# lukefleed/two-pass-lanczos

Measured on AMD Instinct MI355X. Metric: Lanczos iterations/sec + SpMV GB/s (vs HBM roofline), 500k-arc KKT k=500, higher is better.
Workload: dtype f64

## Files before the change

two-pass-lanczos_amd/csrc/tpl_k_p2_fused.hip:

```cpp
#include "tpl_klaunch.h"

namespace tpl {

constexpr int kHubAhead = 8;

struct FusedP2Args {
  const int32_t* h_row;
  const int32_t* h_ent;
  const double* h_val;
  int32_t n_open, n_hub;
  double* ycache;
  const double* rec;
  const int32_t* flags;
  const double* v1;
  double* x;
  int64_t n;
  int32_t n_long;
  int32_t steps;
  const void* s_col;
  const void* s_val;
  const int32_t* s_cbase;
  const int32_t* c_base;
  const int32_t* c_width;
  int32_t n_short, n_chunks, s_width, val_i8, s_col16;
};

__device__ __forceinline__ int fused_steps(const FusedP2Args& a) {
  if (a.steps > 0) return a.steps;
  return a.flags[1] || a.flags[4] ? 0 : a.flags[2];
}

struct StepRec {
  double beta_sub, alpha, invb, ycoef;
};
__device__ __forceinline__ StepRec rec_fields(double cv) {
  return {readlane_f64(cv, 0), readlane_f64(cv, 1), readlane_f64(cv, 2), readlane_f64(cv, 3)};
}
__device__ __forceinline__ void fused_step_r(double s, const StepRec& r, double& vc, double& vp,
                                             double& xv) {
  double w = s - r.beta_sub * vp;
  w = w - r.alpha * vc;
  const double vn = w * r.invb;
  xv = xv + r.ycoef * vn;
  vp = vc;
  vc = vn;
}
__device__ __forceinline__ void fused_step(double s, double cv, double& vc, double& vp, double& xv) {
  fused_step_r(s, rec_fields(cv), vc, vp, xv);
}

constexpr uint32_t kLaneOff = 0x80000000u;
__device__ __forceinline__ void st_cache_row(double* row, int nl, uint32_t off, double v) {
  typedef uint32_t u32x2 __attribute__((ext_vector_type(2)));
  const __amdgpu_buffer_rsrc_t r = __builtin_amdgcn_make_buffer_rsrc(row, 0, nl * 8, 0x00020000);
  u32x2 d;
  d.x = (uint32_t)__double2loint(v);
  d.y = (uint32_t)__double2hiint(v);
  __builtin_amdgcn_raw_buffer_store_b64(d, r, off, 0, 0);
}

enum HubMode { kHubLong, kHubLds, kHubWave };
constexpr int kWave = 64;
template <HubMode MODE>
__device__ __forceinline__ void hub_chain(const FusedP2Args& a, double (*vh)[kTPB], int last,
                                          int lc, bool writes, bool open,
                                          const int (&ent)[kFusedWidth],
                                          const double (&av)[kFusedWidth], double& vc, double& vp,
                                          double& xv) {
  const int t = threadIdx.x;
  const int nl = a.n_long;
  double yb[kHubAhead], cb[kHubAhead];
#pragma unroll
  for (int u = 0; u < kHubAhead; ++u) {
    const int jj = clampi(1 + u, last);
    yb[u] = a.ycache[(size_t)(jj - 1) * nl + lc];
    cb[u] = a.rec[8 * (size_t)jj + (t & 7)];
  }
  const uint32_t soff = writes ? (uint32_t)lc * 8u : kLaneOff;
  auto step = [&](int j, double s, double cv) {
    st_cache_row(a.ycache + (size_t)(j - 1) * nl, nl, soff, vc);
    if (MODE == kHubLds) {
      double* vb = vh[j & 1];
      vb[t] = vc;
      __syncthreads();
      if (open) {
        s = 0.0;
#pragma unroll
        for (int k = 0; k < kFusedWidth; ++k) {
          const double prod = av[k] * vb[ent[k] < 0 ? 0 : ent[k]];
          s = s + (ent[k] >= 0 ? prod : -0.0);
        }
      }
    }
    if (MODE == kHubWave) {
      double so = 0.0;
#pragma unroll
      for (int k = 0; k < kFusedWidth; ++k) {
        const double prod = av[k] * __shfl(vc, ent[k] < 0 ? 0 : ent[k], kWave);
        so = so + (ent[k] >= 0 ? prod : -0.0);
      }
      s = open ? so : s;
    }
    fused_step(s, cv, vc, vp, xv);
  };
  const int nblk = last / kHubAhead;
  int j0 = 1;
  if (nblk > 0) __builtin_amdgcn_s_waitcnt(0x0F70);
  for (int b = 0; b < nblk; ++b, j0 += kHubAhead) {
#pragma unroll
    for (int u = 0; u < kHubAhead; ++u) {
      const int j = j0 + u;
      step(j, yb[u], cb[u]);
      __builtin_amdgcn_sched_barrier(0);
      const int jn = clampi(j + kHubAhead, last);
      yb[u] = a.ycache[(size_t)(jn - 1) * nl + lc];
      cb[u] = a.rec[8 * (size_t)jn + (t & 7)];
    }
  }
  const int rem = last - nblk * kHubAhead;
#pragma unroll
  for (int u = 0; u < kHubAhead - 1; ++u) {
    if (u >= rem) break;
    step(j0 + u, yb[u], cb[u]);
  }
}

__global__ __launch_bounds__(kTPB) void k_p2_hub(FusedP2Args a) {
  __shared__ double vh[2][kTPB];
  const int steps = fused_steps(a);
  if (steps < 2) return;
  const int last = steps - 1;
  const int t = threadIdx.x;
  const int nl = a.n_long;
  const int64_t first_long = a.n - nl;
  const int n_lb = (nl + kTPB - 1) / kTPB;
  const bool hub = (int)blockIdx.x >= n_lb;
  bool live, open = false;
  int lc;
  int64_t row;
  int ent[kFusedWidth];
  double av[kFusedWidth];
#pragma unroll
  for (int k = 0; k < kFusedWidth; ++k) {
    ent[k] = -1;
    av[k] = 0.0;
  }
  if (hub) {
    live = t < a.n_hub;
    open = t < a.n_open;
    row = a.h_row[clampi(t, a.n_hub - 1)];
    lc = open ? 0 : clampi((int)(row - first_long), nl - 1);
    if (open) {
#pragma unroll
      for (int k = 0; k < kFusedWidth; ++k) {
        ent[k] = a.h_ent[t * kFusedWidth + k];
        av[k] = a.h_val[t * kFusedWidth + k];
      }
    }
  } else {
    const int l = blockIdx.x * kTPB + t;
    lc = clampi(l, nl - 1);
    row = first_long + lc;
    live = l < nl;
    for (int h = a.n_open; h < a.n_hub; ++h) live = live && a.h_row[h] != (int32_t)row;
  }
  double vc = a.v1[row], vp = 0.0, xv = a.x[row];
  if (hub && a.n_hub <= kWave) {
    if (t >= kWave) return;
    hub_chain<kHubWave>(a, vh, last, lc, live && !open, open, ent, av, vc, vp, xv);
  } else if (hub) {
    hub_chain<kHubLds>(a, vh, last, lc, live && !open, open, ent, av, vc, vp, xv);
  } else {
    hub_chain<kHubLong>(a, vh, last, lc, live, false, ent, av, vc, vp, xv);
  }
  if (live) st_out(a.x + row, xv);
}

__device__ __forceinline__ int fused_col(const FusedP2Args& a, int e, int cbase) {
  if (a.s_col16) {
    const int off = reinterpret_cast<const uint16_t*>(a.s_col)[e];
    return off == 0xFFFF ? -1 : cbase + off;
  }
  return reinterpret_cast<const int32_t*>(a.s_col)[e];
}
__device__ __forceinline__ double fused_val(const FusedP2Args& a, int e) {
  if (a.val_i8) return (double)reinterpret_cast<const int8_t*>(a.s_val)[e];
  return reinterpret_cast<const double*>(a.s_val)[e];
}

constexpr int kRowsGroup = 4;
constexpr int kRowsThreads = kTPB * kRowsGroup;
constexpr int kRowsDepth = 2;

template <int W, int NL>
__global__ __launch_bounds__(kRowsThreads) void k_p2_rows(FusedP2Args a) {
  extern __shared__ double lds[];
  constexpr int NLC = (NL + kRowsGroup - 1) / kRowsGroup;
  constexpr int D = kRowsDepth;
  const int steps = fused_steps(a);
  if (steps < 2) return;
  const int last = steps - 1;
  const int tw = threadIdx.x;
  const int t = tw % kTPB;
  const int chunk_w = blockIdx.x * kRowsGroup + tw / kTPB;
  const bool have = chunk_w < a.n_chunks;
  const int chunk = have ? chunk_w : a.n_chunks - 1;
  const int nl = a.n_long;
  const int first_long = (int)(a.n - nl);
  const int wc = a.s_width > 0 ? a.s_width : a.c_width[chunk];
  const int base = a.s_width > 0 ? chunk * kChunkRows * a.s_width : a.c_base[chunk];
  const bool packed = a.s_width > 0 && packed_chunk_width(a.s_width);
  const int cbase = a.s_col16 ? a.s_cbase[chunk] : 0;
  int row[kRowsPerThread];
  bool live[kRowsPerThread];
  int li[kRowsPerThread][W];
  double av[kRowsPerThread][W];
  double vc[kRowsPerThread], vp[kRowsPerThread], xv[kRowsPerThread];
#pragma unroll
  for (int q = 0; q < kRowsPerThread; ++q) {
    const int p = chunk * kChunkRows + q * kTPB + t;
    live[q] = have && p < a.n_short;
    row[q] = clampi(p, a.n_short - 1);
#pragma unroll
    for (int k = 0; k < W; ++k) {
      const int kc = clampi(k, wc - 1);
      const int e = wc <= 0 ? 0
                    : packed ? base + t * (kRowsPerThread * wc) + q * wc + kc
                             : base + kc * kChunkRows + q * kTPB + t;
      const int c = fused_col(a, e, cbase);
      av[q][k] = fused_val(a, e);
      int idx = -1;
      if (k < wc && c >= 0) {
        if (c >= first_long) idx = c - first_long;
        else if (c == row[q]) idx = -2;
        else live[q] = false;
      }
      li[q][k] = idx;
    }
    vc[q] = a.v1[row[q]];
    vp[q] = 0.0;
    xv[q] = a.x[row[q]];
  }
  double st[D][NLC], cvr[D];
#pragma unroll
  for (int d = 0; d < D; ++d) {
    const int jj = clampi(1 + d, last);
#pragma unroll
    for (int u = 0; u < NLC; ++u)
      st[d][u] = a.ycache[(size_t)(jj - 1) * nl + clampi(tw + u * kRowsThreads, nl - 1)];
    cvr[d] = a.rec[8 * (size_t)jj + (tw & 7)];
  }
  auto step = [&](int j, int d, auto refill) {
    double* vb = lds + (j & 1) * nl;
#pragma unroll
    for (int u = 0; u < NLC; ++u)
      if (u < NLC - 1 || tw + u * kRowsThreads < nl) vb[tw + u * kRowsThreads] = st[d][u];
    const StepRec r = rec_fields(cvr[d]);
    if (decltype(refill)::value) {
      __builtin_amdgcn_sched_barrier(0);
      const int jn = clampi(j + D, last);
#pragma unroll
      for (int u = 0; u < NLC; ++u)
        st[d][u] = a.ycache[(size_t)(jn - 1) * nl + clampi(tw + u * kRowsThreads, nl - 1)];
      cvr[d] = a.rec[8 * (size_t)jn + (tw & 7)];
    }
    __syncthreads();
#pragma unroll
    for (int q = 0; q < kRowsPerThread; ++q) {
      double s = 0.0;
#pragma unroll
      for (int k = 0; k < W; ++k) {
        const double g = vb[li[q][k] < 0 ? 0 : li[q][k]];
        const double prod = av[q][k] * (li[q][k] == -2 ? vc[q] : g);
        s = s + (li[q][k] != -1 ? prod : -0.0);
      }
      fused_step_r(s, r, vc[q], vp[q], xv[q]);
    }
  };
  const int nblk = last / D;
  int j0 = 1;
  if (nblk > 0) __builtin_amdgcn_s_waitcnt(0x0F70);
  for (int b = 0; b < nblk; ++b, j0 += D) {
#pragma unroll
    for (int d = 0; d < D; ++d) step(j0 + d, d, std::true_type{});
  }
  const int rem = last - nblk * D;
#pragma unroll
  for (int d = 0; d < D - 1; ++d) {
    if (d >= rem) break;
    step(j0 + d, d, std::false_type{});
  }
#pragma unroll
  for (int q = 0; q < kRowsPerThread; ++q)
    if (live[q]) st_out(a.x + row[q], xv[q]);
}

namespace launch {

static FusedP2Args fused_args(const CsrDev& A, const DevState& S, const double* ycache,
                              const double* v1, double* x, int steps) {
  FusedP2Args a{};
  a.ycache = const_cast<double*>(ycache);
  a.rec = S.p2c;
  a.flags = S.flags;
  a.v1 = v1;
  a.x = x;
  a.n = A.n;
  a.n_long = A.n_long;
  a.steps = steps;
  a.s_col = A.s_col;
  a.s_val = A.s_val;
  a.s_cbase = A.s_cbase;
  a.c_base = A.c_base;
  a.c_width = A.c_width;
  a.n_short = A.n_short;
  a.n_chunks = A.n_chunks;
  a.s_width = A.s_width;
  a.val_i8 = A.val_i8;
  a.s_col16 = A.s_col16;
  return a;
}

hipError_t p2_fused_hub(const CsrDev& A, const DevState& S, const FusedP2Dev& H, double* ycache,
                        const double* v1, double* x, int steps, hipStream_t s) {
  if (A.n_long <= 0 || !A.s_identity || H.n_hub > kFusedHubMax || H.n_open > H.n_hub)
    return hipErrorInvalidConfiguration;
  FusedP2Args a = fused_args(A, S, ycache, v1, x, steps);
  a.h_row = H.h_row;
  a.h_ent = H.h_ent;
  a.h_val = H.h_val;
  a.n_open = H.n_open;
  a.n_hub = H.n_hub;
  const int grid = (A.n_long + kTPB - 1) / kTPB + (H.n_hub > 0 ? 1 : 0);
  hipLaunchKernelGGL(k_p2_hub, dim3(grid), dim3(kTPB), 0, s, a);
  return hipGetLastError();
}

template <int W, int... NLs>
static bool rows_nl(int nloads, const FusedP2Args& a, int grid, size_t lds, hipStream_t s,
                    std::integer_sequence<int, NLs...>) {
  auto one = [&](auto NL) {
    if (nloads != decltype(NL)::value + 1) return false;
    hipLaunchKernelGGL((k_p2_rows<W, decltype(NL)::value + 1>), dim3(grid), dim3(kRowsThreads),
                       lds, s, a);
    return true;
  };
  return (one(std::integral_constant<int, NLs>{}) || ...);
}

hipError_t p2_fused_rows(const CsrDev& A, const DevState& S, const double* ycache,
                         const double* v1, double* x, int steps, hipStream_t s) {
  if (A.n_long <= 0 || A.n_long > kFusedLongMax || !A.s_identity)
    return hipErrorInvalidConfiguration;
  if (A.n_chunks <= 0) return hipSuccess;
  const FusedP2Args a = fused_args(A, S, ycache, v1, x, steps);
  const size_t lds = 2 * (size_t)A.n_long * sizeof(double);
  const int nloads = (A.n_long + kTPB - 1) / kTPB;
  constexpr auto nls = std::make_integer_sequence<int, kFusedLongMax / kTPB>{};
  const int w = A.s_width > 0 ? A.s_width : kFusedWidth;
  const int grid = (A.n_chunks + kRowsGroup - 1) / kRowsGroup;
  bool ok = false;
  switch (w) {
    case 1: ok = rows_nl<1>(nloads, a, grid, lds, s, nls); break;
    case 2: ok = rows_nl<2>(nloads, a, grid, lds, s, nls); break;
    case 3: ok = rows_nl<3>(nloads, a, grid, lds, s, nls); break;
    case 4: ok = rows_nl<4>(nloads, a, grid, lds, s, nls); break;
    default: break;
  }
  return ok ? hipGetLastError() : hipErrorInvalidConfiguration;
}

}
}
```

Before: 92400.

## Batch several Lanczos steps per LDS sync and specialize hub gather by width

```diff
diff --git a/two-pass-lanczos_amd/csrc/tpl_k_p2_fused.hip b/two-pass-lanczos_amd/csrc/tpl_k_p2_fused.hip
--- a/two-pass-lanczos_amd/csrc/tpl_k_p2_fused.hip
+++ b/two-pass-lanczos_amd/csrc/tpl_k_p2_fused.hip
@@ -33,8 +33,10 @@
 struct StepRec {
   double beta_sub, alpha, invb, ycoef;
 };
-__device__ __forceinline__ StepRec rec_fields(double cv) {
-  return {readlane_f64(cv, 0), readlane_f64(cv, 1), readlane_f64(cv, 2), readlane_f64(cv, 3)};
+__device__ __forceinline__ StepRec rec_scalar(const double* rec, int j) {
+  typedef const double __attribute__((address_space(4))) cdouble;
+  cdouble* p = (cdouble*)(uintptr_t)(rec + 8 * (size_t)j);
+  return {p[0], p[1], p[2], p[3]};
 }
 __device__ __forceinline__ void fused_step_r(double s, const StepRec& r, double& vc, double& vp,
                                              double& xv) {
@@ -45,9 +47,6 @@
   vp = vc;
   vc = vn;
 }
-__device__ __forceinline__ void fused_step(double s, double cv, double& vc, double& vp, double& xv) {
-  fused_step_r(s, rec_fields(cv), vc, vp, xv);
-}
 
 constexpr uint32_t kLaneOff = 0x80000000u;
 __device__ __forceinline__ void st_cache_row(double* row, int nl, uint32_t off, double v) {
@@ -59,9 +58,10 @@
   __builtin_amdgcn_raw_buffer_store_b64(d, r, off, 0, 0);
 }
 
-enum HubMode { kHubLong, kHubLds, kHubWave };
+enum HubMode { kHubLong, kHubLds, kHubWave, kHubLanes };
 constexpr int kWave = 64;
-template <HubMode MODE>
+constexpr int kHubLanesMax = 3;
+template <HubMode MODE, int WM = kFusedWidth, int NH = 0>
 __device__ __forceinline__ void hub_chain(const FusedP2Args& a, double (*vh)[kTPB], int last,
                                           int lc, bool writes, bool open,
                                           const int (&ent)[kFusedWidth],
@@ -69,15 +69,21 @@
                                           double& xv) {
   const int t = threadIdx.x;
   const int nl = a.n_long;
-  double yb[kHubAhead], cb[kHubAhead];
+  double yb[kHubAhead];
+  double2 ra[kHubAhead], rb[kHubAhead];
+  auto load_rec = [&](int u, int jj) {
+    const double2* p = reinterpret_cast<const double2*>(a.rec + 8 * (size_t)jj);
+    ra[u] = p[0];
+    rb[u] = p[1];
+  };
 #pragma unroll
   for (int u = 0; u < kHubAhead; ++u) {
     const int jj = clampi(1 + u, last);
     yb[u] = a.ycache[(size_t)(jj - 1) * nl + lc];
-    cb[u] = a.rec[8 * (size_t)jj + (t & 7)];
+    load_rec(u, jj);
   }
   const uint32_t soff = writes ? (uint32_t)lc * 8u : kLaneOff;
-  auto step = [&](int j, double s, double cv) {
+  auto step = [&](int j, double s, const StepRec& r) {
     st_cache_row(a.ycache + (size_t)(j - 1) * nl, nl, soff, vc);
     if (MODE == kHubLds) {
       double* vb = vh[j & 1];
@@ -86,7 +92,7 @@
       if (open) {
         s = 0.0;
 #pragma unroll
-        for (int k = 0; k < kFusedWidth; ++k) {
+        for (int k = 0; k < WM; ++k) {
           const double prod = av[k] * vb[ent[k] < 0 ? 0 : ent[k]];
           s = s + (ent[k] >= 0 ? prod : -0.0);
         }
@@ -95,14 +101,30 @@
     if (MODE == kHubWave) {
       double so = 0.0;
 #pragma unroll
-      for (int k = 0; k < kFusedWidth; ++k) {
+      for (int k = 0; k < WM; ++k) {
         const double prod = av[k] * __shfl(vc, ent[k] < 0 ? 0 : ent[k], kWave);
         so = so + (ent[k] >= 0 ? prod : -0.0);
       }
       s = open ? so : s;
     }
-    fused_step(s, cv, vc, vp, xv);
-  };
+    if (MODE == kHubLanes) {
+      double bm[NH > 0 ? NH : 1];
+#pragma unroll
+      for (int m = 0; m < NH; ++m) bm[m] = readlane_f64(vc, m);
+      double so = 0.0;
+#pragma unroll
+      for (int k = 0; k < WM; ++k) {
+        double g = bm[0];
+#pragma unroll
+        for (int m = 1; m < NH; ++m) g = ent[k] == m ? bm[m] : g;
+        const double prod = av[k] * g;
+        so = so + (ent[k] >= 0 ? prod : -0.0);
+      }
+      s = open ? so : s;
+    }
+    fused_step_r(s, r, vc, vp, xv);
+  };
+  auto rec_of = [&](int u) { return StepRec{ra[u].x, ra[u].y, rb[u].x, rb[u].y}; };
   const int nblk = last / kHubAhead;
   int j0 = 1;
   if (nblk > 0) __builtin_amdgcn_s_waitcnt(0x0F70);
@@ -110,18 +132,29 @@
 #pragma unroll
     for (int u = 0; u < kHubAhead; ++u) {
       const int j = j0 + u;
-      step(j, yb[u], cb[u]);
+      step(j, yb[u], rec_of(u));
       __builtin_amdgcn_sched_barrier(0);
       const int jn = clampi(j + kHubAhead, last);
       yb[u] = a.ycache[(size_t)(jn - 1) * nl + lc];
-      cb[u] = a.rec[8 * (size_t)jn + (t & 7)];
+      load_rec(u, jn);
     }
   }
   const int rem = last - nblk * kHubAhead;
 #pragma unroll
   for (int u = 0; u < kHubAhead - 1; ++u) {
     if (u >= rem) break;
-    step(j0 + u, yb[u], cb[u]);
+    step(j0 + u, yb[u], rec_of(u));
+  }
+}
+
+template <int NH, typename... Args>
+__device__ __forceinline__ void hub_wave(int wm, Args&&... args) {
+  constexpr HubMode M = NH > 0 ? kHubLanes : kHubWave;
+  switch (wm) {
+    case 1: return hub_chain<M, 1, NH>(args...);
+    case 2: return hub_chain<M, 2, NH>(args...);
+    case 3: return hub_chain<M, 3, NH>(args...);
+    default: return hub_chain<M, kFusedWidth, NH>(args...);
   }
 }
 
@@ -167,7 +200,17 @@
   double vc = a.v1[row], vp = 0.0, xv = a.x[row];
   if (hub && a.n_hub <= kWave) {
     if (t >= kWave) return;
-    hub_chain<kHubWave>(a, vh, last, lc, live && !open, open, ent, av, vc, vp, xv);
+    int wm = 1;
+#pragma unroll
+    for (int k = 1; k < kFusedWidth; ++k)
+      if (__builtin_amdgcn_ballot_w64(ent[k] >= 0) != 0) wm = k + 1;
+    const bool wr = live && !open;
+    static_assert(kHubLanesMax == 3, "the cases below");
+    switch (a.n_hub <= kHubLanesMax ? a.n_hub : 0) {
+      case 2: hub_wave<2>(wm, a, vh, last, lc, wr, open, ent, av, vc, vp, xv); break;
+      case 3: hub_wave<3>(wm, a, vh, last, lc, wr, open, ent, av, vc, vp, xv); break;
+      default: hub_wave<0>(wm, a, vh, last, lc, wr, open, ent, av, vc, vp, xv); break;
+    }
   } else if (hub) {
     hub_chain<kHubLds>(a, vh, last, lc, live && !open, open, ent, av, vc, vp, xv);
   } else {
@@ -191,12 +234,22 @@
 constexpr int kRowsGroup = 4;
 constexpr int kRowsThreads = kTPB * kRowsGroup;
 constexpr int kRowsDepth = 2;
+constexpr int kRowsStepsMax = 3;
+constexpr int kRowsGatherMax = 12;
+
+constexpr int rows_block_steps(int NL) {
+  const int fit = (64 * 1024) / (2 * kTPB * NL * (int)sizeof(double));
+  return fit < kRowsStepsMax ? fit : kRowsStepsMax;
+}
 
 template <int W, int NL>
 __global__ __launch_bounds__(kRowsThreads) void k_p2_rows(FusedP2Args a) {
   extern __shared__ double lds[];
-  constexpr int NLC = (NL + kRowsGroup - 1) / kRowsGroup;
+  constexpr int S = rows_block_steps(NL);
+  constexpr int NLB = (S * NL + kRowsGroup - 1) / kRowsGroup;
   constexpr int D = kRowsDepth;
+  constexpr int kBuf = S * kTPB * NL;
+  static_assert(S >= 1 && 2 * kBuf * sizeof(double) <= 64 * 1024, "two buffers in one workgroup's LDS");
   const int steps = fused_steps(a);
   if (steps < 2) return;
   const int last = steps - 1;
@@ -241,54 +294,126 @@
     vp[q] = 0.0;
     xv[q] = a.x[row[q]];
   }
-  double st[D][NLC], cvr[D];
-#pragma unroll
-  for (int d = 0; d < D; ++d) {
-    const int jj = clampi(1 + d, last);
-#pragma unroll
-    for (int u = 0; u < NLC; ++u)
-      st[d][u] = a.ycache[(size_t)(jj - 1) * nl + clampi(tw + u * kRowsThreads, nl - 1)];
-    cvr[d] = a.rec[8 * (size_t)jj + (tw & 7)];
-  }
-  auto step = [&](int j, int d, auto refill) {
-    double* vb = lds + (j & 1) * nl;
-#pragma unroll
-    for (int u = 0; u < NLC; ++u)
-      if (u < NLC - 1 || tw + u * kRowsThreads < nl) vb[tw + u * kRowsThreads] = st[d][u];
-    const StepRec r = rec_fields(cvr[d]);
+  const int bw = S * nl;
+  bool any_live = false, lane_clean = true;
+#pragma unroll
+  for (int q = 0; q < kRowsPerThread; ++q) {
+    any_live = any_live || live[q];
+#pragma unroll
+    for (int k = 0; k < W; ++k) lane_clean = lane_clean && (!live[q] || k >= wc || li[q][k] >= 0);
+  }
+  const int wcu = __builtin_amdgcn_readfirstlane(wc);
+  const bool idle = __builtin_amdgcn_ballot_w64(any_live) == 0;
+  const bool clean = __builtin_amdgcn_ballot_w64(!lane_clean) == 0;
+  int lx[kRowsPerThread][W];
+#pragma unroll
+  for (int q = 0; q < kRowsPerThread; ++q)
+#pragma unroll
+    for (int k = 0; k < W; ++k) lx[q][k] = (li[q][k] < 0 ? 0 : li[q][k]) * S;
+  double st[D][NLB];
+  int wofs[NLB];
+#pragma unroll
+  for (int u = 0; u < NLB; ++u) {
+    const int i = tw + u * kRowsThreads;
+    int sb = 0;
+#pragma unroll
+    for (int s = 1; s < S; ++s) sb += i >= s * nl ? 1 : 0;
+    wofs[u] = (i - sb * nl) * S + sb;
+  }
+  uint32_t cb[NLB];
+#pragma unroll
+  for (int u = 0; u < NLB; ++u) cb[u] = 8u * (uint32_t)clampi(tw + u * kRowsThreads, bw - 1);
+  auto fill = [&](int d, int b) {
+    int r0 = b * S;
+    if (r0 >= last) r0 = 0;
+    const int rows = clampi(last - r0, S);
+    const uint32_t lim = 8u * (uint32_t)(rows * nl - 1);
+    const char* run = reinterpret_cast<const char*>(a.ycache + (size_t)r0 * nl);
+#pragma unroll
+    for (int u = 0; u < NLB; ++u)
+      st[d][u] = *reinterpret_cast<const double*>(run + (cb[u] < lim ? cb[u] : lim));
+  };
+#pragma unroll
+  for (int d = 0; d < D; ++d) fill(d, d);
+  StepRec rn{};
+  if (!idle) rn = rec_scalar(a.rec, 1);
+  auto row_steps = [&](const double* vb, int b, auto cnt, auto wcc) {
+    constexpr int WC = decltype(wcc)::value;
+    constexpr bool kAhead = WC >= 1 && WC * S * kRowsPerThread <= kRowsGatherMax;
+    double g[kAhead ? S : 1][kRowsPerThread][kAhead ? WC : 1];
+    if constexpr (kAhead) {
+#pragma unroll
+      for (int q = 0; q < kRowsPerThread; ++q)
+#pragma unroll
+        for (int k = 0; k < WC; ++k)
+#pragma unroll
+          for (int s = 0; s < S; ++s) g[s][q][k] = vb[lx[q][k] + s];
+      __builtin_amdgcn_sched_barrier(0);
+    }
+#pragma unroll
+    for (int s = 0; s < S; ++s) {
+      if (s >= cnt) break;
+      const StepRec r = rn;
+      double sum[kRowsPerThread];
+#pragma unroll
+      for (int q = 0; q < kRowsPerThread; ++q) {
+        sum[q] = 0.0;
+        if constexpr (kAhead) {
+#pragma unroll
+          for (int k = 0; k < WC; ++k) sum[q] = sum[q] + av[q][k] * g[s][q][k];
+        } else if constexpr (WC >= 0) {
+#pragma unroll
+          for (int k = 0; k < WC; ++k) sum[q] = sum[q] + av[q][k] * vb[lx[q][k] + s];
+        } else {
+#pragma unroll
+          for (int k = 0; k < W; ++k) {
+            const double g = vb[lx[q][k] + s];
+            const double prod = av[q][k] * (li[q][k] == -2 ? vc[q] : g);
+            sum[q] = sum[q] + (li[q][k] != -1 ? prod : -0.0);
+          }
+        }
+      }
+      __builtin_amdgcn_sched_barrier(0);
+      rn = rec_scalar(a.rec, clampi(2 + b * S + s, last));
+#pragma unroll
+      for (int q = 0; q < kRowsPerThread; ++q) fused_step_r(sum[q], r, vc[q], vp[q], xv[q]);
+    }
+  };
+  auto block = [&](int b, int d, auto cnt, auto refill) {
+    double* vb = lds + (b & 1) * kBuf;
+#pragma unroll
+    for (int u = 0; u < NLB; ++u)
+      if ((u + 1) * kRowsThreads <= S * (kTPB * (NL - 1) + 1) || tw + u * kRowsThreads < bw)
+        vb[wofs[u]] = st[d][u];
     if (decltype(refill)::value) {
       __builtin_amdgcn_sched_barrier(0);
-      const int jn = clampi(j + D, last);
-#pragma unroll
-      for (int u = 0; u < NLC; ++u)
-        st[d][u] = a.ycache[(size_t)(jn - 1) * nl + clampi(tw + u * kRowsThreads, nl - 1)];
-      cvr[d] = a.rec[8 * (size_t)jn + (tw & 7)];
+      fill(d, b + D);
     }
     __syncthreads();
-#pragma unroll
-    for (int q = 0; q < kRowsPerThread; ++q) {
-      double s = 0.0;
-#pragma unroll
-      for (int k = 0; k < W; ++k) {
-        const double g = vb[li[q][k] < 0 ? 0 : li[q][k]];
-        const double prod = av[q][k] * (li[q][k] == -2 ? vc[q] : g);
-        s = s + (li[q][k] != -1 ? prod : -0.0);
-      }
-      fused_step_r(s, r, vc[q], vp[q], xv[q]);
-    }
-  };
-  const int nblk = last / D;
-  int j0 = 1;
-  if (nblk > 0) __builtin_amdgcn_s_waitcnt(0x0F70);
-  for (int b = 0; b < nblk; ++b, j0 += D) {
-#pragma unroll
-    for (int d = 0; d < D; ++d) step(j0 + d, d, std::true_type{});
-  }
-  const int rem = last - nblk * D;
-#pragma unroll
-  for (int d = 0; d < D - 1; ++d) {
-    if (d >= rem) break;
-    step(j0 + d, d, std::false_type{});
+    if (idle) return;
+    if (!clean) return row_steps(vb, b, cnt, std::integral_constant<int, -1>{});
+    switch (wcu) {
+      case 1: return row_steps(vb, b, cnt, std::integral_constant<int, 1>{});
+      case 2: return row_steps(vb, b, cnt, std::integral_constant<int, W < 2 ? W : 2>{});
+      case 3: return row_steps(vb, b, cnt, std::integral_constant<int, W < 3 ? W : 3>{});
+      case 4: return row_steps(vb, b, cnt, std::integral_constant<int, W < 4 ? W : 4>{});
+      default: return row_steps(vb, b, cnt, std::integral_constant<int, 0>{});
+    }
+  };
+  constexpr int B = D * S;
+  const int ngrp = last / B;
+  int b0 = 0;
+  if (ngrp > 0) __builtin_amdgcn_s_waitcnt(0x0F70);
+  for (int g = 0; g < ngrp; ++g, b0 += D) {
+#pragma unroll
+    for (int d = 0; d < D; ++d) block(b0 + d, d, std::integral_constant<int, S>{}, std::true_type{});
+  }
+  const int rem = last - ngrp * B;
+#pragma unroll
+  for (int d = 0; d < D; ++d) {
+    const int cnt = rem - d * S;
+    if (cnt <= 0) break;
+    block(b0 + d, d, cnt, std::false_type{});
   }
 #pragma unroll
   for (int q = 0; q < kRowsPerThread; ++q)
@@ -354,8 +479,8 @@
     return hipErrorInvalidConfiguration;
   if (A.n_chunks <= 0) return hipSuccess;
   const FusedP2Args a = fused_args(A, S, ycache, v1, x, steps);
-  const size_t lds = 2 * (size_t)A.n_long * sizeof(double);
   const int nloads = (A.n_long + kTPB - 1) / kTPB;
+  const size_t lds = (size_t)rows_block_steps(nloads) * (nloads * kTPB + A.n_long) * sizeof(double);
   constexpr auto nls = std::make_integer_sequence<int, kFusedLongMax / kTPB>{};
   const int w = A.s_width > 0 ? A.s_width : kFusedWidth;
   const int grid = (A.n_chunks + kRowsGroup - 1) / kRowsGroup;
```

New measurement: 93420, median of 6. 1.1% higher.
